# tensorflow/compression

Measured on AMD Instinct MI355X. Metric: Mpixels/s encode+decode round-trip (bit-exact), higher is better.
Workload: dtype int32

## Files before the change

compression_amd/_lib.py:

```python
from __future__ import annotations

import ctypes as C
import os

_HERE = os.path.dirname(os.path.abspath(__file__))
LIB_PATH = os.path.join(_HERE, "libtfc_hip.so")

_vp = C.c_void_p
_i64 = C.c_int64
_int = C.c_int

SIGNATURES = {
    "tfc_abi_version": (_int, []),
    "tfc_last_error": (C.c_char_p, []),
    "tfc_profile_enable": (None, [_int]),
    "tfc_set_default_mode": (_int, [_int]),
    "tfc_get_default_mode": (_int, []),
    "tfc_set_chip_shared": (_int, [_int]),
    "tfc_image_to_unit": (_int, [_vp, _vp, _int, C.c_int64, _vp]),
    "tfc_unit_to_image": (_int, [_vp, _int, _vp, C.c_int64, _vp]),
    "tfc_index_prepare": (_int, [_vp, _int, _vp, C.c_int64, _int, _vp]),
    "tfc_build_tables": (_int, [_vp, C.c_int64, C.c_int64, _vp, _vp, C.c_int64, _int, _vp, _vp]),
    "tfc_build_tables_overflow": (_int, [_vp, C.c_int64, C.c_int64, _vp, _vp, C.c_int64, _int, _vp, _vp, _vp]),
    "tfc_deep_factorized_tails": (_int, [_vp, C.c_int64, C.c_int64, _int, _int, _vp, _int, _vp, _vp, _vp]),
    "tfc_pad2d": (_int, [_vp, _vp, _int, C.c_int64, C.c_int64, C.c_int64, C.c_int64, _int, _int, _int, _int, _int, _vp]),
    "tfc_cache_bytes": (_int, [C.POINTER(C.c_longlong)]),
    "tfc_cache_trim": (_int, [C.POINTER(C.c_longlong)]),
    "tfc_encoder_capacity": (_int, [_vp, C.POINTER(_i64)]),
    "tfc_profile_query": (_int, [C.c_char_p, C.POINTER(C.c_double), C.POINTER(_i64)]),
    "tfc_pipe_counters": (_int, [C.POINTER(_i64), C.POINTER(_i64)]),
    "tfc_set_pipe_format": (_int, [_int, _int]),
    "tfc_tables_create": (_int, [_vp, _int, _i64, _i64, _vp, C.POINTER(_vp)]),
    "tfc_tables_count": (_i64, [_vp]),
    "tfc_tables_destroy": (None, [_vp]),
    "tfc_encoder_create": (_int, [_vp, _i64, _vp, C.POINTER(_vp)]),
    "tfc_encoder_create_many": (_int, [_vp, _i64, _int, _vp, _vp]),
    "tfc_encoder_set_mode": (_int, [_vp, _int]),
    "tfc_encoder_set_deferred_errors": (_int, [_vp, _int]),
    "tfc_encoder_encode": (_int, [_vp, _vp, _vp, _i64, _vp]),
    "tfc_encoder_encode_many": (_int, [_int, _vp, _vp, _vp, _i64, _vp]),
    "tfc_encoder_encode_quantized": (_int, [_vp, _vp, _int, _vp, _vp, _i64, _i64, _vp]),
    "tfc_encoder_encode_quantized_indexed": (_int, [_vp, _vp, _int, _vp, _vp, _i64, _vp]),
    "tfc_encoder_encode_quantized_many": (_int, [_int, _vp, _vp, _int, _vp, _vp, _i64, _i64, _vp]),
    "tfc_decoder_decode_dequantized_many": (_int, [_int, _vp, _vp, _int, _vp, _vp, _i64, _i64, _vp]),
    "tfc_encoder_encode_quantized_indexed_many": (_int, [_int, _vp, _vp, _int, _vp, _vp, _i64, _vp]),
    "tfc_decoder_decode_dequantized_indexed_many": (_int, [_int, _vp, _vp, _vp, _int, _vp, _i64, _vp]),
    "tfc_encoder_finalize": (_int, [_vp, _vp, C.POINTER(_i64)]),
    "tfc_encoder_finalize_device": (_int, [_vp, _vp]),
    "tfc_encoder_finalize_device_many": (_int, [_int, _vp, _vp]),
    "tfc_encoder_status": (_int, [_vp, _vp, C.POINTER(_i64)]),
    "tfc_encoder_result": (_int, [_vp, C.POINTER(_vp), C.POINTER(_vp)]),
    "tfc_encoder_read": (_int, [_vp, _vp, _vp, _int, _vp]),
    "tfc_encoder_destroy": (None, [_vp]),
    "tfc_decoder_create": (_int, [_vp, _vp, _vp, _i64, _int, _vp, C.POINTER(_vp)]),
    "tfc_decoder_create_many": (_int, [_vp, _int, _vp, _vp, _vp]),
    "tfc_decoder_set_mode": (_int, [_vp, _int]),
    "tfc_decoder_decode": (_int, [_vp, _vp, _vp, _i64, _vp]),
    "tfc_decoder_decode_many": (_int, [_int, _vp, _vp, _vp, _i64, _vp]),
    "tfc_decoder_decode_dequantized": (_int, [_vp, _vp, _vp, _int, _vp, _vp, _i64, _i64, _vp]),
    "tfc_decoder_finalize": (_int, [_vp, _vp, _vp]),
    "tfc_decoder_finalize_device": (_int, [_vp, _vp, _vp]),
    "tfc_decoder_finalize_device_many": (_int, [_int, _vp, _vp, _vp]),
    "tfc_decoder_status": (_int, [_vp, _vp]),
    "tfc_decoder_destroy": (None, [_vp]),
# ... 129 lines not shown
```

compression_amd/csrc/range_coder.hip:

```cpp
#include <hip/hip_bf16.h>
#include <hip/hip_fp16.h>
#include <hip/hip_runtime.h>

#include <algorithm>
#include <atomic>
#include <cstdlib>
#include <chrono>
#include <cstring>
#include <functional>
#include <type_traits>
#include <memory>
#include <mutex>
#include <string>
#include <vector>

#include "../../include/tfc_hip.h"
#include "common.h"
#include "range_coder_device.h"

namespace tfc {

std::string& last_error() {
  static thread_local std::string e;
  return e;
// ... 1439 lines not shown
  const int64_t ntab = static_cast<int64_t>(t->rows.size());
  if (has_index && (idx < 0 || idx >= ntab))
    return fail("index=%d not in range [0, %lld)", idx, static_cast<long long>(ntab));
  const int2 row = t->rows[has_index ? idx : channel];
  return fail("value=%d not in range [0, %d)", value, row.y - 2);
}

int encoder_error(tfc_encoder* e, const unsigned long long* host_status) {
  e->poisoned = true;
  const unsigned long long pos = host_status[0];
  const int64_t ch = static_cast<int64_t>((pos % static_cast<unsigned long long>(std::max<int64_t>(e->elems_last, 1))) %
                                          e->tables->rows.size());
  return range_error_text(e->tables, e->indexed_last, static_cast<int32_t>(static_cast<long long>(host_status[2])),
                          ch, static_cast<int32_t>(static_cast<long long>(host_status[1])));
}

std::atomic<int>& pipe_format_value() {
  static std::atomic<int> v{[] {
    const char* e = std::getenv("TFC_PIPE_FORMAT");
    if (!e) return 0;
    if (std::strcmp(e, "full") == 0) return 1;
    if (std::strcmp(e, "pairs") == 0) return 2;
    return 0;
  }()};
  return v;
}
std::atomic<int>& pipe_waves_value() {
  static std::atomic<int> v{[] {
    const char* e = std::getenv("TFC_PIPE_WAVES");
    return e ? std::max(0, std::atoi(e)) : 0;
  }()};
  return v;
}
inline int pipe_format() { return pipe_format_value().load(std::memory_order_relaxed); }
inline int pipe_waves_env() { return pipe_waves_value().load(std::memory_order_relaxed); }

inline bool pipe_enabled() {
  static const bool on = [] {
    const char* e = std::getenv("TFC_PIPE");
    return !e || std::atoi(e) != 0;
  }();
  return on;
}
inline bool pipe_fallback_launch() {
  static const bool on = [] {
    const char* e = std::getenv("TFC_PIPE_NOFALLBACK");
    return !e || std::atoi(e) == 0;
  }();
  return on;
}
std::atomic<long long> g_pipe_launches{0};

inline int pipe_overlap() {
  static const int v = [] {
    const char* e = std::getenv("TFC_PIPE_OVERLAP");
    return e ? std::atoi(e) : 2;
  }();
  return v;
}
inline long long pipe_poll_ticks() {
  static const long long v = [] {
    const char* e = std::getenv("TFC_PIPE_POLL_MS");
    return static_cast<long long>(e ? std::atoi(e) : 250) * 100000;
  }();
  return v;
}
// ... 611 lines not shown
    f.job[k].state = es[k]->state.as<uint4>();
    f.job[k].chunk = ChunkRef{c.data.as<uint8_t>(), c.off.as<long long>(), c.len_p, c.stride};
  }
  hipLaunchKernelGGL(enc_tail_many_kernel, dim3(static_cast<unsigned>(ceil_div(streams, 256)), static_cast<unsigned>(n)),
                     dim3(256), 0, st, f);
  hipLaunchKernelGGL(scan_lengths_many_kernel, dim3(static_cast<unsigned>(n)), dim3(1024), 0, st, f);
  hipLaunchKernelGGL(enc_pack_many_kernel,
                     dim3(static_cast<unsigned>(ceil_div(streams, kWavesPerBlock)), static_cast<unsigned>(n)),
                     dim3(kBlock), 0, st, f);
  TFC_HIP(hipGetLastError());
  for (int k = 0; k < n; ++k) {
    tfc_encoder* e = es[k];
    e->result_group = group;
    e->offsets.p = f.base + k * f.job_bytes + f.offsets_off;
    e->blob.p = f.base + k * f.job_bytes + f.blob_off;
    e->blob_capacity = static_cast<int64_t>(cap);
    e->chunks.clear();
    e->finalized = true;
  }
  return 0;
}

extern "C" int tfc_debug_pipe_clocks(unsigned long long* out8) {
  TFC_HIP(hipDeviceSynchronize());
  TFC_HIP(hipMemcpyFromSymbol(out8, HIP_SYMBOL(tfc::g_pipe_clock), 8 * sizeof(unsigned long long)));
  return 0;
}
extern "C" int tfc_debug_enc_clocks(unsigned long long* out4) {
  TFC_HIP(hipDeviceSynchronize());
  TFC_HIP(hipMemcpyFromSymbol(out4, HIP_SYMBOL(tfc::g_enc_clock), 4 * sizeof(unsigned long long)));
  return 0;
}

extern "C" int tfc_pipe_counters(int64_t* launches, int64_t* fallback_blocks) {
  if (launches) *launches = g_pipe_launches.load();
  if (fallback_blocks) {
    unsigned long long v = 0;
    TFC_HIP(hipDeviceSynchronize());
    TFC_HIP(hipMemcpyFromSymbol(&v, HIP_SYMBOL(tfc::g_pipe_fallback_blocks), sizeof(v)));
    *fallback_blocks = static_cast<int64_t>(v);
  }
  return 0;
}

extern "C" int tfc_set_pipe_format(int format, int waves_per_workgroup) {
  if (format < 0 || format > 2 || waves_per_workgroup < 0 || waves_per_workgroup > 8) {
    tfc::fail("tfc_set_pipe_format: format 0 ... 2, waves per workgroup 0 ... 8");
    return -1;
  }
  pipe_waves_value().store(waves_per_workgroup);
  return pipe_format_value().exchange(format);
}

extern "C" int tfc_encoder_set_mode(tfc_encoder* e, int mode) {
  if (mode != TFC_MODE_AUTO && mode != TFC_MODE_LATENCY && mode != TFC_MODE_THROUGHPUT)
    return fail("unknown mode %d", mode);
  if (e->family >= 0) return fail("the mode of a handle is fixed by its first coding call");
  e->mode = mode;
  return 0;
}

extern "C" int tfc_encoder_set_deferred_errors(tfc_encoder* e, int on) {
  e->deferred = on != 0;
  return 0;
}

extern "C" int tfc_encoder_encode(tfc_encoder* e, const int32_t* value, const int32_t* index,
                                  int64_t elems, void* stream) {
  const SymInt32 src{value};
  return encode_jobs(&e, 1, &src, &index, elems, static_cast<hipStream_t>(stream), "tfc_encoder_encode");
}

extern "C" int tfc_encoder_encode_many(int n, tfc_encoder* const* es, const int32_t* const* values,
                                       const int32_t* const* indexes, int64_t elems, void* stream) {
  if (n <= 0) return 0;
  std::vector<SymInt32> srcs(n);
  for (int k = 0; k < n; ++k) srcs[k] = SymInt32{values[k]};
  return encode_jobs(es, n, srcs.data(), indexes, elems, static_cast<hipStream_t>(stream), "tfc_encoder_encode_many");
}

extern "C" int tfc_encoder_encode_quantized(tfc_encoder* e, const void* y, int dtype,
                                            const float* qoffset, const int32_t* cdf_offset,
                                            int64_t channels, int64_t elems, void* stream) {
  if (check_channels(e->tables, channels)) return 1;
// ... 380 lines not shown
  const int64_t rows64 = ((elems + (t->any_escape ? elems / 4 + 64 + 24 * kPipeBlock : 2 * kPipeBlock)) + kPipeBlock - 1) / kPipeBlock * kPipeBlock;
  pa.rows = static_cast<int>(std::min<int64_t>(rows64, (int64_t{1} << 30)));
  const size_t raw_bytes = static_cast<size_t>(pa.rows) * 128;
  const size_t rec_bytes = (static_cast<size_t>(pa.rows) / kPipeBlock + 1) * 256;
  const size_t group_bytes = raw_bytes + rec_bytes + 64 * sizeof(uint4) + sizeof(unsigned int);
  const size_t job_bytes = group_bytes * pa.groups_per_job + (indexed ? 2 * static_cast<size_t>(streams) * elems : 0);
  pla.lds_wave = (indexed ? PipeDecLds::kBytes : PipeDecLds::kRows) + PipeDecLds::kStage;
  const size_t kPipeTempBytes = pipe_temp_bytes();
  const int cus_d = pipe_device_info().cus;
  const int64_t waves_call = static_cast<int64_t>(pa.groups_per_job) * std::min(n, kMaxLaneJobs);
  auto waves_fit = [&](int image_bytes) { return std::max(0, (160 * 1024 - image_bytes) / pla.lds_wave); };
  const int pair_image = (t->pair_dec_bytes + 1023) & ~1023;
  const int fit_full = waves_fit(pla.lds_image), fit_pairs = t->pairs_ok ? waves_fit(pair_image) : 0;
  bool pairs = false;
  switch (pipe_format()) {
    case 1: pairs = false; break;
    case 2: pairs = fit_pairs >= 1; break;
    default: pairs = fit_pairs >= 1 && (fit_full < 1 || 4 * waves_call > 3 * static_cast<int64_t>(cus_d) * std::min(fit_full, 4));
  }
  if (pairs) {
    pla.image = t->d_pair_image.as<uint32_t>();
    pla.bytes = t->pair_dec_bytes;
    pla.lds_image = pair_image;
  }
  const int fit = pairs ? fit_pairs : fit_full;
  int per = static_cast<int>(std::min<int64_t>(8, std::max<int64_t>(1, ceil_div(waves_call, static_cast<int64_t>(cus_d)))));
  if (g_chip_shared.load(std::memory_order_relaxed) != 0) per = std::max(per, static_cast<int>(std::min<int64_t>(4, pa.groups_per_job)));
  if (pipe_waves_env() > 0) per = pipe_waves_env();
  per = std::min(per, std::min(fit, pa.groups_per_job));
  const int pblock = 64 * std::max(per, 0);
  const bool pipe = pipe_enabled() && pblock >= 64 && rows64 < (int64_t{1} << 30) && job_bytes <= kPipeTempBytes &&
                    (!indexed || la.ntab < 4096) && t->lane_precision <= 15 &&
                    (static_cast<int64_t>(pa.rows) / kParseRows + 1) * pa.groups_per_job * kMaxLaneJobs < (int64_t{1} << 31);
  const int plds = pla.lds_image + (pblock / 64) * pla.lds_wave;
  const size_t chain_wgs_per_job = static_cast<size_t>(ceil_div(pa.groups_per_job, std::max(1, pblock / 64)));
  const size_t resident_wgs = static_cast<size_t>(cus_d) * std::max<size_t>(1, (160 * 1024) / std::max(1, plds));
  const size_t resident_jobs = std::max<size_t>(1, resident_wgs / std::max<size_t>(1, chain_wgs_per_job));
  const int per_launch = !pipe ? kMaxLaneJobs
                               : static_cast<int>(std::max<size_t>(1, std::min<size_t>(std::min<size_t>(kMaxLaneJobs, resident_jobs),
                                                                                      kPipeTempBytes / std::max<size_t>(job_bytes, 1))));
  const void* pfn = nullptr;
  if (pipe) {
    pfn = pairs ? (indexed ? reinterpret_cast<const void*>(&dec_chain_kernel<true, true>) : reinterpret_cast<const void*>(&dec_chain_kernel<false, true>))
                : (indexed ? reinterpret_cast<const void*>(&dec_chain_kernel<true, false>) : reinterpret_cast<const void*>(&dec_chain_kernel<false, false>));
    TFC_HIP(hipFuncSetAttribute(pfn, hipFuncAttributeMaxDynamicSharedMemorySize, plds));
  }
  if (!pipe && !lanes_fit) {
    for (int k = 0; k < n; ++k) {
      KernelTimer timer("dec_kernel", st);
      if (launch_wave_decoder(ds[k], indexed ? indexes[k] : nullptr, elems, dsts[k], st, nullptr)) return 1;
    }
    return 0;
  }
  const PipePairMap pm{t->d_pair_adjust.as<int>()};
  for (int g0 = 0; g0 < n; g0 += per_launch) {
    const int gn = std::min(per_launch, n - g0);
    DecLaneJobs<Dst> jobs;
    jobs.streams = streams;
    jobs.elems = elems;
    jobs.blocks_per_job = static_cast<int>(ceil_div(streams, block));
    jobs.n = gn;
    for (int k = 0; k < gn; ++k) {
      tfc_decoder* d = ds[g0 + k];
      DecLaneJob<Dst>& J = jobs.job[k];
      J.dst = dsts[g0 + k];
      J.index = indexed ? indexes[g0 + k] : nullptr;
      J.blob = d->blob_p;
// ... 3 lines not shown
    }
    KernelTimer timer("dec_kernel", st);
    DevBuf temp;
    bool piped = pipe;
    la.guard = nullptr;
    if (pipe) do {
      const size_t groups = static_cast<size_t>(pa.groups_per_job) * gn;
      const size_t tiles = static_cast<size_t>(pa.rows) / kParseRows + 1;
      const size_t raw_all = raw_bytes * groups, rec_all = rec_bytes * groups, st_all = 64 * sizeof(uint4) * groups;
      const size_t kend_all = (sizeof(unsigned int) * groups + 255) & ~size_t{255};
      const size_t addr_all = indexed ? ((2 * static_cast<size_t>(streams) * elems * gn + 255) & ~size_t{255}) : 0;
      const size_t flags_all = (512 + sizeof(unsigned int) * groups * (1 + tiles) + 255) & ~size_t{255};
      if (temp.alloc(raw_all + rec_all + st_all + kend_all + addr_all + flags_all, st) != hipSuccess) {
        (void)hipGetLastError();
        temp.p = nullptr;
        piped = false;
        break;
      }
      uint8_t* base = temp.as<uint8_t>();
      pa.raw = reinterpret_cast<unsigned short*>(base);
      pa.posrec = reinterpret_cast<unsigned int*>(base + raw_all);
      pa.state_out = reinterpret_cast<uint4*>(base + raw_all + rec_all);
      pa.kend = reinterpret_cast<unsigned int*>(base + raw_all + rec_all + st_all);
      unsigned short* rowaddr = reinterpret_cast<unsigned short*>(base + raw_all + rec_all + st_all + kend_all);
      pa.rowaddr = rowaddr;
      pa.fallback = reinterpret_cast<unsigned int*>(base + raw_all + rec_all + st_all + kend_all + addr_all);
      pa.started = pa.fallback + 64;
      pa.progress = pa.fallback + 128;
      pa.tile_done = pa.progress + groups;
      pa.groups = static_cast<int>(groups);
      pa.poll_ticks = 200000;
      TFC_HIP(hipMemsetAsync(pa.fallback, 0, flags_all, st));
      g_pipe_launches.fetch_add(1, std::memory_order_relaxed);
      PipeDecJobs cj;
      cj.streams = streams;
      cj.elems = elems;
      cj.blocks_per_job = static_cast<int>(ceil_div(pa.groups_per_job, pblock / 64));
      cj.n = gn;
      for (int k = 0; k < gn; ++k) cj.job[k] = PipeDecJob{jobs.job[k].blob, jobs.job[k].off, jobs.job[k].state};
      if (indexed) {
        PipeRowJobs rj;
        rj.per_job = streams * elems;
        rj.ntab = la.ntab;
        rj.n = gn;
        for (int k = 0; k < gn; ++k) { rj.job[k].index = jobs.job[k].index; rj.job[k].first_error = jobs.job[k].first_error; }
        hipLaunchKernelGGL(dec_rows_kernel, dim3(static_cast<unsigned>(ceil_div(rj.per_job, 1024)), static_cast<unsigned>(gn)),
                           dim3(256), 0, st, rj, rowaddr);
      }
      const int overlap = groups >= 64 ? pipe_overlap() : 0;
      SideStream side;
      if (overlap) {
        if (side_stream(st, &side)) return 1;
        TFC_HIP(hipEventRecord(side.fork, st));
        TFC_HIP(hipStreamWaitEvent(side.stream, side.fork, 0));
      }
      const hipStream_t cst = overlap ? side.stream : st;
      const dim3 cgrid(static_cast<unsigned>(cj.blocks_per_job * gn));
      const dim3 pgrid(static_cast<unsigned>(groups * tiles));
      const size_t ctiles = std::min<size_t>(tiles, static_cast<size_t>(ceil_div(elems, static_cast<int64_t>(kParseRows))));
      const dim3 pgrid_next(static_cast<unsigned>(groups * ctiles));
      {
        KernelTimer t2("dec_chain", cst);
        if (pairs && indexed) hipLaunchKernelGGL((dec_chain_kernel<true, true>), cgrid, dim3(pblock), plds, cst, cj, pla, pa);
        else if (pairs) hipLaunchKernelGGL((dec_chain_kernel<false, true>), cgrid, dim3(pblock), plds, cst, cj, pla, pa);
        else if (indexed) hipLaunchKernelGGL((dec_chain_kernel<true, false>), cgrid, dim3(pblock), plds, cst, cj, pla, pa);
        else hipLaunchKernelGGL((dec_chain_kernel<false, false>), cgrid, dim3(pblock), plds, cst, cj, pla, pa);
// ... 759 lines not shown
```

compression_amd/csrc/range_pipe.h:

```cpp
#pragma once

#ifndef TFC_PIPE_TIMING
#define TFC_PIPE_TIMING 0
#endif

namespace tfc {

constexpr int kPipeTile = 256;
constexpr int kPipeEscMax = 32;
constexpr unsigned int kPipeBlock = 16;
constexpr unsigned int kPipeNoCall = 0x0001FFFFu;
constexpr unsigned int kPipeAggregate = 1u << 30;
constexpr unsigned int kPipePrefix = 2u << 30;
constexpr unsigned int kPipeRowsMask = (1u << 30) - 1u;

struct PipeEncArgs {
  const uint16_t* fast16;
  const int2* rows_fast;
  int ntab;
  int tab_entries;
  unsigned int* calls;
  unsigned int* status;
  unsigned int* done;
  unsigned int* fallback;
// ... 826 lines not shown
  const unsigned int job = gi / static_cast<unsigned int>(pa.groups_per_job);
  const unsigned int gidx = gi % static_cast<unsigned int>(pa.groups_per_job);
  if (pa.fallback[job] != 0u) return;
  const int64_t s = static_cast<int64_t>(gidx) * 64 + threadIdx.x;
  if (s >= jobs.streams) return;
  const PipeChainJob& J = jobs.job[job];
  J.state[s] = pa.stage_state[static_cast<size_t>(gi) * 64 + threadIdx.x];
  const uint2 o = pa.stage_out[static_cast<size_t>(gi) * 64 + threadIdx.x];
  J.chunk_len[s] = o.y ? 0u : o.x;
  if (o.y) atomicOr(J.overflow_flag, 1u);
}


constexpr unsigned int kPipeSkipRow = 0xFFFFu;
__device__ inline unsigned int pipe_raw_entry(unsigned int sym_or_bit, int M) { return (M != 0 ? 0x8000u : 0u) | sym_or_bit; }
__device__ inline int pipe_mode_step(int M, unsigned int bit) {
  if (M < 0) return bit ? -M : (M == -31 ? 32 : M - 1);
  return M - 1;
}

struct PipeDecArgs {
  unsigned short* raw;
  unsigned int* posrec;
  unsigned int* kend;
  uint4* state_out;
  const unsigned short* rowaddr;
  unsigned int* fallback;
  unsigned int* progress;
  unsigned int* tile_done;
  unsigned int* started;
  int rows;
  int groups_per_job;
  int groups;
  int concurrent;
  long long poll_ticks;
};
constexpr unsigned int kPipeFinal = 0x80000000u;
#ifndef TFC_PIPE_RELEASE
#define TFC_PIPE_RELEASE 64
#endif
constexpr unsigned int kPipeRelease = TFC_PIPE_RELEASE;
struct PipeDecJob { const uint8_t* blob; const long long* off; const uint4* state; };
struct PipeDecJobs {
  int64_t streams, elems;
  int blocks_per_job, n;
  PipeDecJob job[64];
};

struct PipeRowJobs {
  int64_t per_job;
  int ntab, n;
  struct { const int32_t* index; unsigned long long* first_error; } job[64];
};
__global__ void __launch_bounds__(256) dec_rows_kernel(const PipeRowJobs jobs, unsigned short* rowaddr) {
  const int k = blockIdx.y;
  const int32_t* index = jobs.job[k].index;
  unsigned short* out = rowaddr + static_cast<size_t>(k) * jobs.per_job;
  for (int64_t i = static_cast<int64_t>(blockIdx.x) * 1024 + threadIdx.x, e = min(jobs.per_job, (static_cast<int64_t>(blockIdx.x) + 1) * 1024);
       i < e; i += 256) {
    int t = tfc_gload(index + i);
    if (t < 0 || t >= jobs.ntab) {
      atomicMin(jobs.job[k].first_error, static_cast<unsigned long long>(i));
      t = 0;
    }
    out[i] = static_cast<unsigned short>(16 * t);
  }
}

struct PipeDecLds {
  static constexpr int kWords = 2 * kPipeBlock * 2 / 8 + 2;
  static constexpr int kStride = lane_stride(8 * kWords);
  static constexpr int kCodes = 0;
  static constexpr int kRows = kCodes + 64 * kStride;
  static constexpr int kBytes = kRows + 64 * kStride;
  static constexpr int kStage = kPipeBlock * 128;
};

#ifndef TFC_PDEC_ABL
#define TFC_PDEC_ABL 0
#endif
#if TFC_PDEC_ABL & 1
#define TFC_PDEC_STORE(KOFF)
#define TFC_PDEC_WAIT2 "s_waitcnt lgkmcnt(1)\n\t"
#else
#define TFC_PDEC_STORE(KOFF) "ds_write_b16 %[STG], v117 offset:" #KOFF "\n\t"
#define TFC_PDEC_WAIT2 "s_waitcnt lgkmcnt(2)\n\t"
#endif
#ifndef TFC_PDEC_PAD
#define TFC_PDEC_PAD 0
#endif
#define TFC_PDEC_PAD2 "v_mov_b32 v139, v139\n\tv_mov_b32 v139, v139\n\t"
#if TFC_PDEC_PAD == 1
#define TFC_PDEC_PAD_A TFC_PDEC_PAD2
#elif TFC_PDEC_PAD == 5
#define TFC_PDEC_PAD_A "s_waitcnt lgkmcnt(15)\n\ts_waitcnt lgkmcnt(15)\n\t"
#else
#define TFC_PDEC_PAD_A
#endif
#if TFC_PDEC_PAD == 2
#define TFC_PDEC_PAD_B TFC_PDEC_PAD2
#else
#define TFC_PDEC_PAD_B
#endif
#if TFC_PDEC_PAD == 3
#define TFC_PDEC_PAD_C TFC_PDEC_PAD2
#else
#define TFC_PDEC_PAD_C
#endif
// ... 170 lines not shown
      if (i + 1u == entries) esclo = 1u << (la.precision - 1);
      else if (esc) esclo = lds_u16(lanes_lds, e->cdf + 2u * limit + 2u) >> (16 - la.precision);
      e->info = limit | (esc << 15) | ((0xFFFFu - esclo) << 16);
      e->bits -= 8u;
      e->cum -= 2u;
      if (i + 1u == entries) e->cdf -= 0x10000u;
    }
    __syncthreads();
  }

  const unsigned long long clk0 = clock64(), wall0 = wall_clock64();
  if (threadIdx.x == 0u) __hip_atomic_fetch_add(pa.started, 1u, __ATOMIC_RELAXED, __HIP_MEMORY_SCOPE_AGENT);
  const unsigned int job = blockIdx.x / static_cast<unsigned int>(jobs.blocks_per_job);
  const unsigned int wv = (blockIdx.x % static_cast<unsigned int>(jobs.blocks_per_job)) * (blockDim.x >> 6) + (threadIdx.x >> 6);
  if (wv >= static_cast<unsigned int>(pa.groups_per_job)) return;
  const unsigned int gi = job * static_cast<unsigned int>(pa.groups_per_job) + wv;
  const PipeDecJob& J = jobs.job[job];
  const unsigned int lane = threadIdx.x & 63u;
  const int64_t s = static_cast<int64_t>(wv) * 64 + lane;
  const bool live = s < jobs.streams;
  const unsigned int elems = live ? static_cast<unsigned int>(jobs.elems) : 0u;

  const uint4 st = live ? J.state[s] : make_uint4(0u, 0xFFFFFFFFu, 0u, 2u);
  unsigned int D = st.z - st.x;
  unsigned int s1 = st.y;
  const long long o0 = live ? J.off[s] : 0;
  unsigned int len = live ? static_cast<unsigned int>(J.off[s + 1] - o0) : 0u;
  unsigned int pos_start = 2u * st.w;
  lanes_pin(D, s1, len, pos_start);

  const unsigned int lds0 = static_cast<unsigned int>(reinterpret_cast<size_t>(
      (__attribute__((address_space(3))) unsigned char*)lanes_lds));
  const unsigned int wave_off = static_cast<unsigned int>(la.lds_image) + (threadIdx.x >> 6) * static_cast<unsigned int>(la.lds_wave);
  LaneWindow<L::kWords> cw;
  const unsigned int cw_off = wave_off + L::kCodes + L::kStride * lane;
  cw.lds = lanes_lds + cw_off;
  cw.g = J.blob + o0;
  cw.len = len;
  cw.request(pos_start);
  cw.base = pos_start;
  unsigned int cp = cw_off;
  LaneWindow<L::kWords> iw;
  const unsigned int iw_off = wave_off + L::kRows + L::kStride * lane;
  if (INDEXED) {
    iw.lds = lanes_lds + iw_off;
    iw.g = reinterpret_cast<const unsigned char*>(pa.rowaddr + (static_cast<size_t>(job) * jobs.streams + (live ? s : 0)) * jobs.elems);
    iw.len = elems * 2u;
    iw.request(0u);
    iw.base = 0u;
  }

  const unsigned int stg_off = wave_off + (INDEXED ? L::kBytes : L::kRows);
  const unsigned int stg = stg_off + 2u * lane;
  bool staged = false;
  unsigned int staged_k = 0u;

  const float scale = static_cast<float>(1u << la.precision);
  float hscale = scale;
  asm volatile("" : "+v"(hscale));
  const unsigned int cp_max = (1u << la.precision) - 1u;
  const unsigned int pair_sh = 16u - static_cast<unsigned int>(la.precision);
  const unsigned int pair_nsh = 0u - (1u << pair_sh);
  const unsigned int dir_end = 16u * static_cast<unsigned int>(la.ntab);
  const unsigned int bin_addr = dir_end + 16u * kLaneDirRepeat;
  uint4 bin = *reinterpret_cast<const uint4*>(lanes_lds + bin_addr);
  asm volatile("" : "+v"(bin.x), "+v"(bin.y), "+v"(bin.z), "+v"(bin.w));
  unsigned int bin_addr_v = bin_addr;
  asm volatile("" : "+v"(bin_addr_v));

  unsigned int pos = 0u;
  int M = 0;
  unsigned int pw = INDEXED ? iw_off : 0u;
  uint4 R = make_uint4(0u, 0u, 0u, 0u);
  bool row_loaded = false;

  unsigned short* const raw = pa.raw + static_cast<size_t>(gi) * pa.rows * 64;
  unsigned int* const posrec = pa.posrec + static_cast<size_t>(gi) * (pa.rows / kPipeBlock + 1) * 64 + lane;
  unsigned int k = 0u;
  auto flush = [&]() {
    if (!staged) return;
#if TFC_PDEC_ABL & 4
    staged = false;
    return;
#endif
    unsigned char* dst = reinterpret_cast<unsigned char*>(raw + static_cast<size_t>(staged_k) * 64) + 16u * lane;
// ... 86 lines not shown
        const unsigned int half = scale16(s1, 32768u);
        const unsigned int bit = D >= half ? 1u : 0u;
        const unsigned int A = bit ? half : 0u;
        const unsigned int b = bit ? s1 : half - 1u;
        D -= A;
        s1 = b - A;
        const bool ren = (s1 >> 16) == 0u;
        D = ren ? (D << 16) | dig : D;
        s1 = ren ? (s1 << 16) | 0xFFFFu : s1;
        cp += ren ? 2u : 0u;
        entry = PAIRS ? 0x8001u + bit : pipe_raw_entry(bit, M);
        if (M < 0) {
          if (bit) M = -M;
          else M = M == -31 ? 32 : M - 1;
        } else {
          --M;
        }
      }
      if (M == 0) {
        ++pos;
        pw += INDEXED ? 2u : 16u;
        if (!INDEXED && pw == dir_end) pw = 0u;
        load_row();
      } else {
        R = bin;
      }
      if (to_stage) *reinterpret_cast<unsigned short*>(lanes_lds + stg + 128u * (row - k)) = static_cast<unsigned short>(entry);
      else raw[static_cast<size_t>(row) * 64 + lane] = static_cast<unsigned short>(entry);
    }
  };

#if TFC_PIPE_TIMING
  unsigned long long t_asm = 0ull, n_asm = 0ull, t_commit = 0ull, t_rest = 0ull;
#endif
  auto memory_phase = [&]() __attribute__((always_inline)) {
#if TFC_PIPE_TIMING
    const unsigned long long tm0 = clock64();
#endif
    const unsigned int cpos = cw.base + (cp - cw_off);
    cw.commit();
    cp = cw_off + (cpos - cw.base);
    if (INDEXED) {
      iw.commit();
      pw = iw_off + (2u * pos - iw.base);
    }
#if TFC_PIPE_TIMING
    asm volatile("s_waitcnt lgkmcnt(0)" ::: "memory");
    const unsigned long long tm1 = clock64();
    t_commit += tm1 - tm0;
#endif
    flush();
    if (k != 0u && (k / kPipeBlock) % kPipeRelease == 0u) {
      posrec[static_cast<size_t>(k / kPipeBlock) * 64] = pos + (M != 0 ? 1u : 0u);
      __builtin_amdgcn_fence(__ATOMIC_RELEASE, "agent");
      if (lane == 0u) __hip_atomic_store(&pa.progress[gi], k, __ATOMIC_RELAXED, __HIP_MEMORY_SCOPE_AGENT);
    }
    cw.request(cpos);
    if (INDEXED) iw.request(2u * pos);
    posrec[static_cast<size_t>(k / kPipeBlock) * 64] = pos + (M != 0 ? 1u : 0u);
#if TFC_PIPE_TIMING
    t_rest += clock64() - tm1;
#endif
  };
  auto fast_block = [&](unsigned int& flag) __attribute__((always_inline)) {
#define TFC_PDEC_OPERANDS                                                                                              \
        : [D] "+v"(D), [S] "+v"(s1), [CP] "+v"(cp), [M] "+v"(M), [PW] "+v"(pw), [FLAG] "+v"(flag),                    \
          [R0] "+v"(R.x), [R1] "+v"(R.y), [R2] "+v"(R.z), [R3] "+v"(R.w)                                              \
        : [STG] "v"(stg), [BINROW] "v"(bin_addr_v), [SCALE] "s"(scale), [HSCALE] "v"(hscale),        \
          [K64K] "s"(0x10000u), [KFFFF] "s"(0xFFFFu), [PERM] "s"(0x05040001u), [NSH] "s"(pair_nsh) \
        : "vcc", "memory", "s52", "s53", "s54", "s55", "s56", "s57", "s58", "s59", "v104", "v105", "v106", "v107", "v108", "v109", "v110", "v111", "v112", "v113", \
          "v114", "v115", "v116", "v117", "v118", "v119", "v122", "v123", "v124", "v125", "v126", "v127", "v128",      \
          "v129", "v130", "v131", "v132", "v133", "v134", "v135", "v136", "v137", "v138", "v139", "v140", "v141", "v142", "v143", "v144", "v145"
#if TFC_PIPE_TIMING
    const unsigned long long ta = clock64();
#endif
    if constexpr (INDEXED && PAIRS) asm volatile(TFC_PDEC_BLOCK(TFC_PDEC_STEP_PIX) TFC_PDEC_OPERANDS);
    else if constexpr (PAIRS) asm volatile(TFC_PDEC_BLOCK(TFC_PDEC_STEP_PCH) TFC_PDEC_OPERANDS);
    else if constexpr (INDEXED) asm volatile(TFC_PDEC_BLOCK(TFC_PDEC_STEP_IX) TFC_PDEC_OPERANDS);
    else asm volatile(TFC_PDEC_BLOCK(TFC_PDEC_STEP_CH) TFC_PDEC_OPERANDS);
#if TFC_PIPE_TIMING
    t_asm += clock64() - ta;
    ++n_asm;
#endif
  };
  auto fast_step = [&](unsigned int& flag, unsigned int slot) __attribute__((always_inline)) {
    const unsigned int stg_row = stg + 128u * slot;
    {
      const unsigned int stg = stg_row;
      if constexpr (INDEXED && PAIRS) asm volatile(TFC_PDEC_ONE(TFC_PDEC_STEP_PIX) TFC_PDEC_OPERANDS);
      else if constexpr (PAIRS) asm volatile(TFC_PDEC_ONE(TFC_PDEC_STEP_PCH) TFC_PDEC_OPERANDS);
      else if constexpr (INDEXED) asm volatile(TFC_PDEC_ONE(TFC_PDEC_STEP_IX) TFC_PDEC_OPERANDS);
      else asm volatile(TFC_PDEC_ONE(TFC_PDEC_STEP_CH) TFC_PDEC_OPERANDS);
    }
#undef TFC_PDEC_OPERANDS
  };
  bool gave_up = false;
  while (__any(pos < elems)) {
    if (lds0 == 0u && row_loaded && (INDEXED || static_cast<unsigned int>(la.ntab) >= kPipeBlock)) {
      while (__all(!live || (pos + kPipeBlock <= elems && M > -16)) && k + kPipeBlock <= static_cast<unsigned int>(pa.rows)) {
        memory_phase();
        const unsigned int D0 = D, s10 = s1, cp0 = cp, pw0 = pw;
        const int M0 = M;
        const uint4 R0 = R;
        unsigned int flag = 0u;
        fast_block(flag);
        if (__builtin_expect(__any(live && flag != 0u), 0)) {
          D = D0; s1 = s10; cp = cp0; pw = pw0; M = M0; R = R0;
#pragma nounroll
          for (unsigned int i = 0; i < kPipeBlock; ++i) {
            const unsigned int D1 = D, s11 = s1, cp1 = cp, pw1 = pw;
            const int M1 = M;
            const uint4 R1 = R;
            unsigned int f1 = 0u;
            if (live) fast_step(f1, i);
            if (__any(live && f1 != 0u)) {
              D = D1; s1 = s11; cp = cp1; pw = pw1; M = M1; R = R1;
              gstep(live, k + i, true);
            } else {
              pos += (pw - pw1) / (INDEXED ? 2u : 16u);
              if (!INDEXED) pw -= pw >= dir_end ? dir_end : 0u;
            }
          }
          staged = true;
          staged_k = k;
          k += kPipeBlock;
          continue;
        }
        pos += (pw - pw0) / (INDEXED ? 2u : 16u);
        if (!INDEXED) pw -= pw >= dir_end ? dir_end : 0u;
        staged = true;
        staged_k = k;
        k += kPipeBlock;
      }
      if (!__any(pos < elems)) break;
    }
    if (k + kPipeBlock > static_cast<unsigned int>(pa.rows)) {
      gave_up = true;
      break;
    }
    memory_phase();
    if (!row_loaded) {
      if (M == 0) load_row(); else R = bin;
      row_loaded = true;
    }
    const bool whole = pos + kPipeBlock <= elems;
    const bool blocks = __any(whole);
    if (blocks && __any(!whole && pos < elems && M != 0)) {
      if (pos < elems) {
#pragma unroll
        for (unsigned int i = 0; i < kPipeBlock; ++i) raw[static_cast<size_t>(k + i) * 64 + lane] = static_cast<unsigned short>(kPipeSkipRow);
      }
#pragma nounroll
      for (unsigned int i = 0; i < kPipeBlock; ++i) gstep(!whole && pos < elems && M != 0, k + i);
      k += kPipeBlock;
      continue;
    }
    const bool busy = blocks ? whole : pos < elems;
    const bool sitting = blocks && !whole && pos < elems;
    if (__builtin_expect(lds0 == 0u && blocks && !__any(busy && M <= -16), 1)) {
      if (__any(sitting)) {
        if (sitting) {
#pragma unroll
          for (unsigned int i = 0; i < kPipeBlock; ++i) *reinterpret_cast<unsigned short*>(lanes_lds + stg + 128u * i) = static_cast<unsigned short>(kPipeSkipRow);
        }
      }
// ... 11 lines not shown
        if (!INDEXED)
          while (__any(busy && pw >= dir_end)) pw -= pw >= dir_end ? dir_end : 0u;
        staged = true;
        staged_k = k;
        k += kPipeBlock;
        continue;
      }
      D = D0; s1 = s10; cp = cp0; pw = pw0; M = M0; R = R0;
    }
    if (sitting) {
#pragma unroll
      for (unsigned int i = 0; i < kPipeBlock; ++i) raw[static_cast<size_t>(k + i) * 64 + lane] = static_cast<unsigned short>(kPipeSkipRow);
    }
#pragma nounroll
    for (unsigned int i = 0; i < kPipeBlock; ++i) gstep(busy && pos < elems, k + i);
    k += kPipeBlock;
  }
  flush();
  posrec[static_cast<size_t>(k / kPipeBlock) * 64] = pos;
  if (gave_up) {
    if (lane == 0) {
      atomicOr(&pa.fallback[job], 1u);
      __hip_atomic_store(&pa.progress[gi], kPipeFinal, __ATOMIC_RELEASE, __HIP_MEMORY_SCOPE_AGENT);
    }
    return;
  }
  if (lane == 0) pa.kend[gi] = k;
  __builtin_amdgcn_fence(__ATOMIC_RELEASE, "agent");
  if (lane == 0) __hip_atomic_store(&pa.progress[gi], k | kPipeFinal, __ATOMIC_RELAXED, __HIP_MEMORY_SCOPE_AGENT);
  if (gi == 0 && lane == 0) {
    g_pipe_clock[2] = clock64() - clk0;
    g_pipe_clock[3] = wall_clock64() - wall0;
#if TFC_PIPE_TIMING
    g_pipe_clock[5] = t_asm | (t_commit << 32);
    g_pipe_clock[7] = n_asm | (static_cast<unsigned long long>(k) << 16) | (t_rest << 32);
#endif
  }
  if (live) {
    const unsigned int cpos = cw.base + (cp - cw_off);
    const unsigned char* srcp = J.blob + o0;
    unsigned int window = 0u;
    for (int i = -4; i < 0; ++i) {
      const long long q = static_cast<long long>(cpos) + i;
      window = (window << 8) | ((q >= 0 && q < static_cast<long long>(len)) ? srcp[q] : 0u);
    }
    pa.state_out[static_cast<size_t>(gi) * 64 + lane] = make_uint4(window - D, s1, window, cpos >> 1);
  }
}

constexpr int kParseRows = 128;
constexpr unsigned int kParseMargin = 96;

constexpr int kParseEscTables = 2048;

struct PipePairMap { const int* adjust; };
template <bool INDEXED, bool PAIRS, typename Dst>
__global__ void __launch_bounds__(256) dec_parse_kernel(const DecLaneJobs<Dst> jobs, const PipeDecArgs pa, const DecRow* dir, int ntab,
                                                        const PipePairMap pm) {
  constexpr int kPitch = 66;
  __shared__ unsigned short buf[kParseRows * kPitch];
  __shared__ unsigned int escsym[kParseEscTables];
  __shared__ unsigned int incomplete;
  const unsigned int tiles = static_cast<unsigned int>(pa.rows) / kParseRows + 1u;
  const unsigned int gi = blockIdx.x % static_cast<unsigned int>(pa.groups), kt = blockIdx.x / static_cast<unsigned int>(pa.groups);
  const unsigned int job = gi / static_cast<unsigned int>(pa.groups_per_job);
  const unsigned int wv = gi % static_cast<unsigned int>(pa.groups_per_job);
  const DecLaneJob<Dst>& J = jobs.job[job];
  const unsigned int tid = threadIdx.x, lane = tid & 63u;
  const unsigned int k0 = kt * kParseRows;
  unsigned int* const tile_done = pa.tile_done + static_cast<size_t>(gi) * tiles + kt;
  unsigned int kend;
  bool final = true;
  if (pa.concurrent) {
    const unsigned int need = k0 + kParseRows + kParseMargin;
    unsigned int* const abandon = pa.started + 1;
    unsigned int v = 0u;
    if (tid == 0u) {
      unsigned int seen = ~0u, go = 1u;
      long long t0 = 0;
      if (__hip_atomic_load(abandon, __ATOMIC_RELAXED, __HIP_MEMORY_SCOPE_AGENT) != 0u) go = 0u;
      while (go) {
        v = __hip_atomic_load(&pa.progress[gi], __ATOMIC_RELAXED, __HIP_MEMORY_SCOPE_AGENT);
        if ((v & kPipeFinal) || v >= need) break;
        const long long now = static_cast<long long>(wall_clock64());
        if (v != seen) { seen = v; t0 = now; }
        else if (now - t0 > pa.poll_ticks) {
// ... 114 lines not shown
```

include/tfc_hip.h:

```cpp
#ifndef TFC_HIP_H_
#define TFC_HIP_H_

#include <stdint.h>

#ifdef __cplusplus
extern "C" {
#endif

typedef struct tfc_tables tfc_tables;
typedef struct tfc_encoder tfc_encoder;
typedef struct tfc_decoder tfc_decoder;

#define TFC_ABI_VERSION 2
int tfc_abi_version(void);
const char* tfc_last_error(void);

void tfc_profile_enable(int on);
int tfc_profile_query(const char* kernel, double* total_ms, int64_t* launches);
int tfc_pipe_counters(int64_t* launches, int64_t* fallback_blocks);
int tfc_set_pipe_format(int format, int waves_per_workgroup);

#define TFC_MODE_AUTO 0
#define TFC_MODE_LATENCY 1
#define TFC_MODE_THROUGHPUT 2
int tfc_set_default_mode(int mode);
int tfc_get_default_mode(void);

int tfc_set_chip_shared(int shared);
int tfc_image_to_unit(const void* x, void* y, int dtype, int64_t n, void* stream);
int tfc_unit_to_image(const void* x, int dtype, void* y, int64_t n, void* stream);
int tfc_index_prepare(const void* indexes, int dtype, int32_t* out, int64_t n, int num_tables, void* stream);
int tfc_pad2d(const void* x, void* y, int elem_bytes, int64_t n, int64_t h, int64_t w, int64_t c, int top, int bottom,
              int left, int right, int reflect, void* stream);
int tfc_cache_bytes(long long* bytes);
int tfc_cache_trim(long long* released);


int tfc_tables_create(const int32_t* lookup, int rank, int64_t rows, int64_t cols,
                      void* stream, tfc_tables** out);
int64_t tfc_tables_count(const tfc_tables* t);
void tfc_tables_destroy(tfc_tables* t);


int tfc_encoder_create(const tfc_tables* tables, int64_t streams, void* stream,
                       tfc_encoder** out);

int tfc_encoder_create_many(const tfc_tables* tables, int64_t streams, int n, void* stream,
                            tfc_encoder** out);

int tfc_encoder_set_mode(tfc_encoder* e, int mode);
int tfc_encoder_set_deferred_errors(tfc_encoder* e, int on);

int tfc_encoder_encode(tfc_encoder* e, const int32_t* value, const int32_t* index,
// ... 259 lines not shown
```

Before: 62310.

## Widen pipelined decoder LDS window to fill spare LDS and skip refills

The pipelined range decoder's per-lane LDS bitstream window can now be larger than the fixed minimum. The host picks the largest window that does not reduce workgroups per CU or parse-kernel co-residency, and it can be capped through an env var or API. The decode loop refills the window only when some live lane is within 66 bytes of its end, instead of at every block. This cuts global loads and LDS commits per block, at the cost of more registers for pending words and a more complex loop structure.

Result: no change. 62220 (-0.2%).

```diff
diff --git a/compression_amd/_lib.py b/compression_amd/_lib.py
--- a/compression_amd/_lib.py
+++ b/compression_amd/_lib.py
@@ -30,6 +30,7 @@
     "tfc_profile_query": (_int, [C.c_char_p, C.POINTER(C.c_double), C.POINTER(_i64)]),
     "tfc_pipe_counters": (_int, [C.POINTER(_i64), C.POINTER(_i64)]),
     "tfc_set_pipe_format": (_int, [_int, _int]),
+    "tfc_set_pipe_window": (_int, [_int]),
     "tfc_tables_create": (_int, [_vp, _int, _i64, _i64, _vp, C.POINTER(_vp)]),
     "tfc_tables_count": (_i64, [_vp]),
     "tfc_tables_destroy": (None, [_vp]),
diff --git a/compression_amd/csrc/range_coder.hip b/compression_amd/csrc/range_coder.hip
--- a/compression_amd/csrc/range_coder.hip
+++ b/compression_amd/csrc/range_coder.hip
@@ -1495,6 +1495,15 @@
   }()};
   return v;
 }
+std::atomic<int>& pipe_window_value() {
+  static std::atomic<int> v{[] {
+    const char* e = std::getenv("TFC_PIPE_WINDOW");
+    const int b = e ? std::atoi(e) : 0;
+    return b >= 8 * PipeDecLds::kWords && b <= 8 * PipeDecLds::kMaxWords ? b : 0;
+  }()};
+  return v;
+}
+std::atomic<int> g_pipe_window_last{0};
 inline int pipe_format() { return pipe_format_value().load(std::memory_order_relaxed); }
 inline int pipe_waves_env() { return pipe_waves_value().load(std::memory_order_relaxed); }
 
@@ -2172,6 +2181,8 @@
   return 0;
 }
 
+extern "C" int tfc_debug_pipe_window() { return g_pipe_window_last.load(); }
+
 extern "C" int tfc_pipe_counters(int64_t* launches, int64_t* fallback_blocks) {
   if (launches) *launches = g_pipe_launches.load();
   if (fallback_blocks) {
@@ -2190,6 +2201,14 @@
   }
   pipe_waves_value().store(waves_per_workgroup);
   return pipe_format_value().exchange(format);
+}
+
+extern "C" int tfc_set_pipe_window(int bytes) {
+  if (bytes != 0 && (bytes < 8 * tfc::PipeDecLds::kWords || bytes > 8 * tfc::PipeDecLds::kMaxWords || bytes % 16 != 0)) {
+    tfc::fail("tfc_set_pipe_window: 0, or a multiple of 16 from %d to %d bytes", 8 * tfc::PipeDecLds::kWords, 8 * tfc::PipeDecLds::kMaxWords);
+    return -1;
+  }
+  return pipe_window_value().exchange(bytes);
 }
 
 extern "C" int tfc_encoder_set_mode(tfc_encoder* e, int mode) {
@@ -2636,7 +2655,23 @@
   const bool pipe = pipe_enabled() && pblock >= 64 && rows64 < (int64_t{1} << 30) && job_bytes <= kPipeTempBytes &&
                     (!indexed || la.ntab < 4096) && t->lane_precision <= 15 &&
                     (static_cast<int64_t>(pa.rows) / kParseRows + 1) * pa.groups_per_job * kMaxLaneJobs < (int64_t{1} << 31);
-  const int plds = pla.lds_image + (pblock / 64) * pla.lds_wave;
+  int plds = pla.lds_image + (pblock / 64) * pla.lds_wave;
+  int win_words = PipeDecLds::kWords;
+  if (pipe) {
+    const int cu_lds = 160 * 1024;
+    const int wgs_cu = cu_lds / plds, parse_cu = std::min(2, (cu_lds - wgs_cu * plds) / kParseLdsBytes);
+    const int limit = pipe_window_value().load(std::memory_order_relaxed);
+    const int top = PipeDecLds::max_words(indexed);
+    const int max_words = limit > 0 ? std::min(limit / 8, top) & ~1 : top;
+    for (int w = PipeDecLds::kWords + 2; w <= max_words; w += 2) {
+      const int lds_w = pla.lds_image + (pblock / 64) * PipeDecLds::wave_bytes(w, indexed);
+      if (lds_w > cu_lds || cu_lds / lds_w != wgs_cu || std::min(2, (cu_lds - wgs_cu * lds_w) / kParseLdsBytes) != parse_cu) break;
+      win_words = w;
+    }
+    pla.lds_wave = PipeDecLds::wave_bytes(win_words, indexed);
+    plds = pla.lds_image + (pblock / 64) * pla.lds_wave;
+  }
+  pa.win_words = win_words;
   const size_t chain_wgs_per_job = static_cast<size_t>(ceil_div(pa.groups_per_job, std::max(1, pblock / 64)));
   const size_t resident_wgs = static_cast<size_t>(cus_d) * std::max<size_t>(1, (160 * 1024) / std::max(1, plds));
   const size_t resident_jobs = std::max<size_t>(1, resident_wgs / std::max<size_t>(1, chain_wgs_per_job));
@@ -2706,6 +2741,7 @@
       pa.poll_ticks = 200000;
       TFC_HIP(hipMemsetAsync(pa.fallback, 0, flags_all, st));
       g_pipe_launches.fetch_add(1, std::memory_order_relaxed);
+      g_pipe_window_last.store(8 * pa.win_words, std::memory_order_relaxed);
       PipeDecJobs cj;
       cj.streams = streams;
       cj.elems = elems;
diff --git a/compression_amd/csrc/range_pipe.h b/compression_amd/csrc/range_pipe.h
--- a/compression_amd/csrc/range_pipe.h
+++ b/compression_amd/csrc/range_pipe.h
@@ -882,6 +882,7 @@
   int rows;
   int groups_per_job;
   int groups;
+  int win_words;
   int concurrent;
   long long poll_ticks;
 };
@@ -919,11 +920,71 @@
 
 struct PipeDecLds {
   static constexpr int kWords = 2 * kPipeBlock * 2 / 8 + 2;
+  static constexpr int kMaxWords = 18, kMaxWordsIndexed = 14;
+  __host__ __device__ static constexpr int max_words(bool indexed) { return indexed ? kMaxWordsIndexed : kMaxWords; }
+  __host__ __device__ static constexpr int stride(int words) { return lane_stride(8 * words); }
   static constexpr int kStride = lane_stride(8 * kWords);
   static constexpr int kCodes = 0;
   static constexpr int kRows = kCodes + 64 * kStride;
   static constexpr int kBytes = kRows + 64 * kStride;
   static constexpr int kStage = kPipeBlock * 128;
+  __host__ __device__ static constexpr int wave_bytes(int words, bool indexed) {
+    return (indexed ? 2 : 1) * 64 * stride(words) + kStage;
+  }
+};
+static_assert(PipeDecLds::kWords % 2 == 0 && PipeDecLds::kMaxWords % 2 == 0 && PipeDecLds::kMaxWordsIndexed % 2 == 0 && PipeDecLds::kWords >= 9, "windows are whole 16-byte loads of at least 72 bytes");
+
+template <int MAXWORDS>
+struct PipeWindow {
+  unsigned char* lds;
+  const unsigned char* g;
+  unsigned int len;
+  unsigned int base;
+  unsigned int pbase;
+  uint2 pend[MAXWORDS];
+
+  __device__ __noinline__ unsigned int tail_word(unsigned int q0) const {
+    unsigned int word = 0u;
+#pragma nounroll
+    for (unsigned int k = 0; k < 4u; ++k)
+      if (q0 + k < len) word |= static_cast<unsigned int>(lanes_gload8(g + q0 + k)) << (8u * k);
+    return word;
+  }
+  __device__ void request(unsigned int pos, int words) {
+    pbase = pos;
+    if (pos + 8u * static_cast<unsigned int>(words) <= len) {
+#pragma unroll
+      for (int w = 0; w < MAXWORDS; w += 2) {
+        if (w < PipeDecLds::kWords || w < words) {
+#if defined(TFC_PDEC_ABL) && (TFC_PDEC_ABL & 2)
+          const uint4 v = w == 0 ? lanes_gload16(g + pos) : make_uint4(pend[0].x, pend[0].y, pend[1].x, pend[1].y);
+#else
+          const uint4 v = lanes_gload16(g + pos + 8u * w);
+#endif
+          pend[w] = make_uint2(v.x, v.y);
+          pend[w + 1] = make_uint2(v.z, v.w);
+        }
+      }
+    } else {
+#pragma unroll
+      for (int w = 0; w < MAXWORDS; ++w) {
+        if (w < PipeDecLds::kWords || w < words) {
+          pend[w].x = tail_word(pos + 8u * w);
+          pend[w].y = tail_word(pos + 8u * w + 4u);
+        }
+      }
+    }
+  }
+  __device__ void commit(int words) {
+#pragma unroll
+    for (int w = 0; w < MAXWORDS; w += 2) {
+      if (w < PipeDecLds::kWords || w < words) {
+        reinterpret_cast<uint2*>(lds)[w] = pend[w];
+        reinterpret_cast<uint2*>(lds)[w + 1] = pend[w + 1];
+      }
+    }
+    base = pbase;
+  }
 };
 
 #ifndef TFC_PDEC_ABL
@@ -1160,25 +1221,29 @@
   const unsigned int lds0 = static_cast<unsigned int>(reinterpret_cast<size_t>(
       (__attribute__((address_space(3))) unsigned char*)lanes_lds));
   const unsigned int wave_off = static_cast<unsigned int>(la.lds_image) + (threadIdx.x >> 6) * static_cast<unsigned int>(la.lds_wave);
-  LaneWindow<L::kWords> cw;
-  const unsigned int cw_off = wave_off + L::kCodes + L::kStride * lane;
+  const int win_words = pa.win_words;
+  const unsigned int win_bytes = 8u * static_cast<unsigned int>(win_words);
+  const unsigned int win_stride = static_cast<unsigned int>(L::stride(win_words));
+  PipeWindow<L::max_words(INDEXED)> cw;
+  const unsigned int cw_off = wave_off + win_stride * lane;
   cw.lds = lanes_lds + cw_off;
   cw.g = J.blob + o0;
   cw.len = len;
-  cw.request(pos_start);
+  cw.request(pos_start, win_words);
   cw.base = pos_start;
   unsigned int cp = cw_off;
-  LaneWindow<L::kWords> iw;
-  const unsigned int iw_off = wave_off + L::kRows + L::kStride * lane;
+  PipeWindow<L::max_words(INDEXED)> iw;
+  const unsigned int iw_off = wave_off + 64u * win_stride + win_stride * lane;
   if (INDEXED) {
     iw.lds = lanes_lds + iw_off;
     iw.g = reinterpret_cast<const unsigned char*>(pa.rowaddr + (static_cast<size_t>(job) * jobs.streams + (live ? s : 0)) * jobs.elems);
     iw.len = elems * 2u;
-    iw.request(0u);
+    iw.request(0u, win_words);
     iw.base = 0u;
   }
-
-  const unsigned int stg_off = wave_off + (INDEXED ? L::kBytes : L::kRows);
+  bool win_pending = true;
+
+  const unsigned int stg_off = wave_off + (INDEXED ? 128u : 64u) * win_stride;
   const unsigned int stg = stg_off + 2u * lane;
   bool staged = false;
   unsigned int staged_k = 0u;
@@ -1331,22 +1396,29 @@
 
 #if TFC_PIPE_TIMING
   unsigned long long t_asm = 0ull, n_asm = 0ull, t_commit = 0ull, t_rest = 0ull;
-#endif
-  auto memory_phase = [&]() __attribute__((always_inline)) {
+  unsigned int n_phase = 0u, n_request = 0u;
+#endif
+  auto phase_commit = [&]() __attribute__((always_inline)) {
 #if TFC_PIPE_TIMING
     const unsigned long long tm0 = clock64();
 #endif
     const unsigned int cpos = cw.base + (cp - cw_off);
-    cw.commit();
+    cw.commit(win_words);
     cp = cw_off + (cpos - cw.base);
     if (INDEXED) {
-      iw.commit();
+      iw.commit(win_words);
       pw = iw_off + (2u * pos - iw.base);
     }
+    win_pending = false;
 #if TFC_PIPE_TIMING
     asm volatile("s_waitcnt lgkmcnt(0)" ::: "memory");
+    t_commit += clock64() - tm0;
+#endif
+  };
+  auto phase_rest = [&]() __attribute__((always_inline)) {
+#if TFC_PIPE_TIMING
     const unsigned long long tm1 = clock64();
-    t_commit += tm1 - tm0;
+    ++n_phase;
 #endif
     flush();
     if (k != 0u && (k / kPipeBlock) % kPipeRelease == 0u) {
@@ -1354,12 +1426,28 @@
       __builtin_amdgcn_fence(__ATOMIC_RELEASE, "agent");
       if (lane == 0u) __hip_atomic_store(&pa.progress[gi], k, __ATOMIC_RELAXED, __HIP_MEMORY_SCOPE_AGENT);
     }
-    cw.request(cpos);
-    if (INDEXED) iw.request(2u * pos);
+    const unsigned int cpos = cw.base + (cp - cw_off);
+    bool is_short = cpos + 66u > cw.base + win_bytes;
+    if (INDEXED) is_short = is_short || 2u * pos + 66u > iw.base + win_bytes;
+    if (__any(live && is_short)) {
+      cw.request(cpos, win_words);
+      if (INDEXED) iw.request(2u * pos, win_words);
+      win_pending = true;
+#if TFC_PIPE_TIMING
+      ++n_request;
+#endif
+    } else if (!live) {
+      cp = cw_off;
+      if (INDEXED) pw = iw_off;
+    }
     posrec[static_cast<size_t>(k / kPipeBlock) * 64] = pos + (M != 0 ? 1u : 0u);
 #if TFC_PIPE_TIMING
     t_rest += clock64() - tm1;
 #endif
+  };
+  auto memory_phase = [&]() __attribute__((always_inline)) {
+    if (win_pending) phase_commit();
+    phase_rest();
   };
   auto fast_block = [&](unsigned int& flag) __attribute__((always_inline)) {
 #define TFC_PDEC_OPERANDS                                                                                              \
@@ -1396,8 +1484,13 @@
   bool gave_up = false;
   while (__any(pos < elems)) {
     if (lds0 == 0u && row_loaded && (INDEXED || static_cast<unsigned int>(la.ntab) >= kPipeBlock)) {
-      while (__all(!live || (pos + kPipeBlock <= elems && M > -16)) && k + kPipeBlock <= static_cast<unsigned int>(pa.rows)) {
-        memory_phase();
+      auto steady = [&]() __attribute__((always_inline)) {
+        return __all(!live || (pos + kPipeBlock <= elems && M > -16)) && k + kPipeBlock <= static_cast<unsigned int>(pa.rows);
+      };
+      while (steady()) {
+        if (win_pending) phase_commit();
+        do {
+        phase_rest();
         const unsigned int D0 = D, s10 = s1, cp0 = cp, pw0 = pw;
         const int M0 = M;
         const uint4 R0 = R;
@@ -1430,6 +1523,7 @@
         staged = true;
         staged_k = k;
         k += kPipeBlock;
+        } while (!win_pending && steady());
       }
       if (!__any(pos < elems)) break;
     }
@@ -1507,6 +1601,8 @@
     g_pipe_clock[2] = clock64() - clk0;
     g_pipe_clock[3] = wall_clock64() - wall0;
 #if TFC_PIPE_TIMING
+    g_pipe_clock[2] = (g_pipe_clock[2] & 0xFFFFFFFFull) | (static_cast<unsigned long long>(n_phase) << 32);
+    g_pipe_clock[3] = (g_pipe_clock[3] & 0xFFFFFFFFull) | (static_cast<unsigned long long>(n_request) << 32);
     g_pipe_clock[5] = t_asm | (t_commit << 32);
     g_pipe_clock[7] = n_asm | (static_cast<unsigned long long>(k) << 16) | (t_rest << 32);
 #endif
@@ -1527,6 +1623,7 @@
 constexpr unsigned int kParseMargin = 96;
 
 constexpr int kParseEscTables = 2048;
+constexpr int kParseLdsBytes = (kParseRows * 66 * 2 + kParseEscTables * 4 + 4 + 511) & ~511;
 
 struct PipePairMap { const int* adjust; };
 template <bool INDEXED, bool PAIRS, typename Dst>
diff --git a/include/tfc_hip.h b/include/tfc_hip.h
--- a/include/tfc_hip.h
+++ b/include/tfc_hip.h
@@ -19,6 +19,7 @@
 int tfc_profile_query(const char* kernel, double* total_ms, int64_t* launches);
 int tfc_pipe_counters(int64_t* launches, int64_t* fallback_blocks);
 int tfc_set_pipe_format(int format, int waves_per_workgroup);
+int tfc_set_pipe_window(int bytes);
 
 #define TFC_MODE_AUTO 0
 #define TFC_MODE_LATENCY 1
```
